# CrystalSixone/VLN-GOAT

Measured on AMD Instinct MI355X. Metric: trajectory-steps/sec fwd+bwd (GOAT pretrain, 36 views x 768, 80 tok), higher is better.
Workload: dtype bf16; 1 GPU; Full R2R GOAT pretrain config (pretrain_src/run_r2r_goat.sh): 6,3,2 layers text/cross/pano, vocab 50265, per-rank batch 48, T=5, 36x768 views, L=80, tasks mlm/sap/cfp 1:1:1, dropout 0.1, fwd+bwd, random-init; global_batch=48, parallelism=dp1, wire=f32, launch=hipGraph replay

## Files before the change

vln-goat_amd/csrc/causal.hip:

```cpp
#include "common.hpp"

namespace {

constexpr int POOL_MAXL = 512;
template <typename T>
__global__ __launch_bounds__(256) void pool_score_kernel(const T* __restrict__ x, const float* __restrict__ w,
                                                         const float* __restrict__ out, const float* __restrict__ dout,
                                                         float* __restrict__ score, int rows, int L, int H,
                                                         const float* __restrict__ smask = nullptr) {
  const int lane = threadIdx.x & 63;
  const int row = blockIdx.x * 4 + (threadIdx.x >> 6);
  if (row >= rows) return;
  const T* xr = x + (int64_t)row * H;
  const int b = row / L;
  float s = 0.f;
  if (out == nullptr) {
    for (int i = lane; i < H; i += 64) s += tanhf(to_f(xr[i])) * w[i];
  } else {
    for (int i = lane; i < H; i += 64) {
      const float o = out[(int64_t)b * H + i];
      s += to_f(xr[i]) * dout[(int64_t)b * H + i] * (1.f - o * o);
    }
  }
  s = wave_sum(s);
// ... 129 lines not shown
    const T* d = dout + (int64_t)row * H;
    const float s = gate[row];
    float dg = 0.f;
    for (int i = lane; i < H; i += 64) dg += to_f(d[i]) * (to_f(a[i]) - to_f(o[i]));
    dg = wave_sum(dg);
    const float dpre = dg * s * (1.f - s);
    pb += dpre;
#pragma unroll
    for (int j = 0; j < DOOR_MAXC; ++j) {
      const int i = lane + 64 * j;
      if (i < H) {
        const float dv = to_f(d[i]), av = to_f(a[i]), ov = to_f(o[i]);
        daug[(int64_t)row * H + i] = from_f<T>(s * dv + dpre * wa[i]);
        dori[(int64_t)row * H + i] = from_f<T>((1.f - s) * dv + dpre * wo[i]);
        pa[j] += dpre * av;
        po[j] += dpre * ov;
      }
    }
  }
#pragma unroll
  for (int j = 0; j < DOOR_MAXC; ++j) {
    const int i = lane + 64 * j;
    if (i < H) { sm[(wave * 2 + 0) * H + i] = pa[j]; sm[(wave * 2 + 1) * H + i] = po[j]; }
  }
  __syncthreads();
  for (int i = threadIdx.x; i < 2 * H; i += 256) {
    const int which = i / H, col = i % H;
    const float v = sm[(0 * 2 + which) * H + col] + sm[(1 * 2 + which) * H + col] + sm[(2 * 2 + which) * H + col] +
                    sm[(3 * 2 + which) * H + col];
    atomicAdd((which ? dwo : dwa) + col, v);
  }
  if (lane == 0) {
    atomicAdd(dbias, pb);
    if (dbias2) atomicAdd(dbias2, pb);
  }
}

template <typename T>
__global__ __launch_bounds__(256) void dict_wsum_fwd_kernel(const float* __restrict__ z, const float* __restrict__ p,
                                                            T* __restrict__ out, int K, int H) {
  const int b = blockIdx.x;
  for (int i = threadIdx.x; i < H; i += 256) {
    float s = 0.f;
    for (int k = 0; k < K; ++k) s += p[(int64_t)b * K + k] * z[((int64_t)b * K + k) * H + i];
    out[(int64_t)b * H + i] = from_f<T>(s);
  }
}
template <typename T>
__global__ __launch_bounds__(256) void dict_wsum_bwd_kernel(const T* __restrict__ dout, const float* __restrict__ z,
                                                            const float* __restrict__ p, float* __restrict__ dz,
                                                            float* __restrict__ dp, int K, int H) {
  const int b = blockIdx.x, lane = threadIdx.x & 63, wave = threadIdx.x >> 6;
  const T* d = dout + (int64_t)b * H;
  if (dz)
    for (int k = 0; k < K; ++k) {
      const float pk = p[(int64_t)b * K + k];
      for (int i = threadIdx.x; i < H; i += 256) dz[((int64_t)b * K + k) * H + i] = pk * to_f(d[i]);
    }
  if (dp)
    for (int k = wave; k < K; k += 4) {
      float s = 0.f;
      for (int i = lane; i < H; i += 64) s += z[((int64_t)b * K + k) * H + i] * to_f(d[i]);
      s = wave_sum(s);
      if (lane == 0) dp[(int64_t)b * K + k] = s;
    }
}


struct NceArgs {
  const float* a[6];
  const float* b[6];
  float* da[6];
  float* db[6];
  float* prob;
  float* loss;
  const float* dloss;
  int Bl, Ba, H, target0;
  float inv_tau;
};

struct NceRole { float* out; int rows; int n; int pd[6]; int is_b[6]; };
struct NceBwdArgs { NceArgs p; NceRole role[8]; int nroles; int row_groups; };

__global__ __launch_bounds__(256) void infonce_fwd_kernel(NceArgs p) {
  extern __shared__ float sh[];
  __shared__ float lsum;
  const int i = blockIdx.x;
  const int lane = threadIdx.x & 63, wave = threadIdx.x >> 6;
  if (threadIdx.x == 0) lsum = 0.f;
  for (int pd = 0; pd < 6; ++pd) {
    const float* arow = p.a[pd] + (int64_t)i * p.H;
    __syncthreads();
    for (int j = wave; j < p.Ba; j += 4) {
      const float* brow = p.b[pd] + (int64_t)j * p.H;
      float s = 0.f;
      for (int k = lane * 4; k < p.H; k += 256) {
        const f32x4 x = *reinterpret_cast<const f32x4*>(arow + k), y = *reinterpret_cast<const f32x4*>(brow + k);
        s += x[0] * y[0] + x[1] * y[1] + x[2] * y[2] + x[3] * y[3];
      }
      s = wave_sum(s);
      if (lane == 0) sh[j] = s * p.inv_tau;
    }
    __syncthreads();
    if (wave == 0) {
      float m = -INFINITY;
      for (int j = lane; j < p.Ba; j += 64) m = fmaxf(m, sh[j]);
      m = wave_max(m);
      float l = 0.f;
      for (int j = lane; j < p.Ba; j += 64) l += __expf(sh[j] - m);
      l = wave_sum(l);
      const float lse = m + __logf(l);
      float* pr = p.prob + ((int64_t)pd * p.Bl + i) * p.Ba;
      for (int j = lane; j < p.Ba; j += 64) pr[j] = __expf(sh[j] - lse);
      if (lane == 0) lsum += 0.5f * (lse - sh[p.target0 + i]);
    }
  }
  __syncthreads();
  if (threadIdx.x == 0) p.loss[i] += lsum;
}

__global__ __launch_bounds__(256) void infonce_bwd_kernel(NceBwdArgs q) {
  const NceArgs& p = q.p;
  const int ro = blockIdx.x / q.row_groups, rg = blockIdx.x % q.row_groups;
  const NceRole& role = q.role[ro];
  const int r = rg * 4 + (threadIdx.x >> 6), c = blockIdx.y * 64 + (threadIdx.x & 63);
  if (r >= role.rows || c >= p.H) return;
  const float half_tau = 0.5f * p.inv_tau;
  float tot = 0.f;
  for (int t = 0; t < role.n; ++t) {
    const int pd = role.pd[t];
    const float* pr = p.prob + (int64_t)pd * p.Bl * p.Ba;
    float acc = 0.f;
    if (!role.is_b[t]) {
      if (r < p.Bl) {
        const float* B = p.b[pd];
        const int tr = p.target0 + r;
        for (int j = 0; j < p.Ba; ++j) acc += (pr[(int64_t)r * p.Ba + j] - (j == tr ? 1.f : 0.f)) * B[(int64_t)j * p.H + c];
        acc *= p.dloss[r] * half_tau;
      }
    } else if (r < p.Ba) {
      const float* A = p.a[pd];
      for (int i = 0; i < p.Bl; ++i)
        acc += (pr[(int64_t)i * p.Ba + r] - (r == p.target0 + i ? 1.f : 0.f)) * (p.dloss[i] * half_tau) * A[(int64_t)i * p.H + c];
    }
    tot += acc;
  }
  role.out[(int64_t)r * p.H + c] += tot;
}


struct SapArgs {
  const void* gs; const void* ls; const void* fwl;
  const uint8_t* gvis; const uint8_t* gvalid; const int64_t* glens; const uint8_t* lmask;
  const float* M; const int64_t* ga; const int64_t* la;
  float* gl; float* ll; float* fused; float* loss; float* lse;
  const float* dloss; const float* dgl; const float* dll; const float* dfused;
  void* dgs; void* dls; void* dfwl;
  int B, G, W, lmask_is_valid, add_stop, fw_sigmoid;
};

__device__ __forceinline__ bool sap_gmasked(const SapArgs& p, int b, int g) {
  bool m = false;
  if (p.gvis) m = m || p.gvis[(int64_t)b * p.G + g] != 0;
  if (p.gvalid) m = m || p.gvalid[(int64_t)b * p.G + g] == 0;
  if (p.glens) m = m || g >= (int)p.glens[b];
  return m;
}
__device__ __forceinline__ bool sap_lmasked(const SapArgs& p, int b, int w) {
  if (!p.lmask) return false;
  const bool v = p.lmask[(int64_t)b * p.W + w] != 0;
  return p.lmask_is_valid ? !v : v;
}
template <typename T>
__device__ __forceinline__ float sap_fw(const SapArgs& p, int b) {
  if (!p.fwl) return 0.5f;
  const float x = (float)reinterpret_cast<const T*>(p.fwl)[b];
  return p.fw_sigmoid ? 1.f / (1.f + __expf(-x)) : x;
}
__device__ __forceinline__ float sap_lse(const float* v, int n, int lane) {
  float m = -INFINITY;
  for (int i = lane; i < n; i += 64) m = fmaxf(m, v[i]);
  m = wave_max(m);
  if (m == -INFINITY) return -INFINITY;
  float s = 0.f;
  for (int i = lane; i < n; i += 64) s += __expf(v[i] - m);
  return m + __logf(wave_sum(s));
}

template <typename T>
__global__ __launch_bounds__(64) void sap_fwd_kernel(SapArgs p) {
  extern __shared__ float sm[];
  float* s_gl = sm; float* s_ll = sm + p.G; float* s_lz = s_ll + p.W; float* s_fu = s_lz + p.W;
  const int b = blockIdx.x, lane = threadIdx.x;
  const float fw = sap_fw<T>(p, b);
  const T* gs = reinterpret_cast<const T*>(p.gs) + (int64_t)b * p.G;
  const T* ls = reinterpret_cast<const T*>(p.ls) + (int64_t)b * p.W;
  for (int g = lane; g < p.G; g += 64) {
    const float v = sap_gmasked(p, b, g) ? -INFINITY : (float)gs[g] * fw;
    s_gl[g] = v;
    p.gl[(int64_t)b * p.G + g] = v;
  }
  for (int w = lane; w < p.W; w += 64) {
    const bool m = sap_lmasked(p, b, w);
    const float r = (float)ls[w] * (1.f - fw);
    s_ll[w] = m ? -INFINITY : r;
    s_lz[w] = m ? 0.f : r;
    p.ll[(int64_t)b * p.W + w] = s_ll[w];
  }
  __syncthreads();
  for (int g = lane; g < p.G; g += 64) {
    float acc = 0.f;
    if (p.M) {
      const float* mr = p.M + ((int64_t)b * p.G + g) * p.W;
      for (int w = 0; w < p.W; ++w) acc += mr[w] * s_lz[w];
    }
    float v = s_gl[g] + acc;
    if (p.add_stop && g == 0) v += s_ll[0];
    s_fu[g] = v;
    p.fused[(int64_t)b * p.G + g] = v;
  }
  __syncthreads();
  if (p.lse) {
    const float lg = sap_lse(s_gl, p.G, lane), lw = sap_lse(s_ll, p.W, lane), lf = sap_lse(s_fu, p.G, lane);
    if (lane == 0) {
      p.lse[b * 3] = lg; p.lse[b * 3 + 1] = lw; p.lse[b * 3 + 2] = lf;
      if (p.loss) {
        const int ga = p.ga ? (int)p.ga[b] : -1, la = p.la ? (int)p.la[b] : -1;
        float l = 0.f;
        if (ga >= 0 && ga < p.G) l += (lg - s_gl[ga]) + (lf - s_fu[ga]);
        if (la >= 0 && la < p.W) l += lw - s_ll[la];
// ... 184 lines not shown
    return 0;
  });
}

extern "C" int goat_door_gate_fwd(void* stream, int dtype, const void* aug, const void* ori, const float* wa,
                                  const float* wo, const float* ba, const float* bo, void* out, float* gate, int rows, int H) {
  if (!aug || !ori || !wa || !wo || !ba || !bo || !out || !gate) return GOAT_E_ARG;
  if (rows <= 0 || H <= 0) return GOAT_E_SHAPE;
  const int blocks = (rows + 3) / 4;
  return dtype_dispatch(dtype, [&](auto dt) -> int {
    typedef GOAT_DT_TYPE(dt) T;
    hipLaunchKernelGGL(door_fwd_kernel<T>, dim3(blocks), dim3(256), 0, ST(stream), (const T*)aug, (const T*)ori, wa, wo, ba, bo,
                       (T*)out, gate, rows, H);
    GOAT_LAUNCH_CHECK();
    return 0;
  });
}

extern "C" int goat_door_gate_bwd(void* stream, int dtype, const void* aug, const void* ori, const float* wa,
                                  const float* wo, const float* gate, const void* dout, void* daug, void* dori, float* dwa,
                                  float* dwo, float* dbias, int rows, int H, float* dbias2) {
  if (!aug || !ori || !wa || !wo || !gate || !dout || !daug || !dori || !dwa || !dwo || !dbias) return GOAT_E_ARG;
  if (rows <= 0 || H <= 0 || H > 64 * DOOR_MAXC) return GOAT_E_SHAPE;
  int blocks = (rows + 3) / 4;
  if (blocks > 256) blocks = 256;
  const size_t sm = (size_t)8 * H * sizeof(float);
  return dtype_dispatch(dtype, [&](auto dt) -> int {
    typedef GOAT_DT_TYPE(dt) T;
    hipLaunchKernelGGL(door_bwd_kernel<T>, dim3(blocks), dim3(256), sm, ST(stream), (const T*)aug, (const T*)ori, wa, wo, gate,
                       (const T*)dout, (T*)daug, (T*)dori, dwa, dwo, dbias, dbias2, rows, H);
    GOAT_LAUNCH_CHECK();
    return 0;
  });
}

extern "C" int goat_dict_wsum_fwd(void* stream, int dtype_out, const float* z, const float* p, void* out, int B, int K,
                                  int H) {
  if (!z || !p || !out) return GOAT_E_ARG;
  if (B <= 0 || K <= 0 || H <= 0) return GOAT_E_SHAPE;
  return dtype_dispatch(dtype_out, [&](auto dt) -> int {
    typedef GOAT_DT_TYPE(dt) T;
    hipLaunchKernelGGL(dict_wsum_fwd_kernel<T>, dim3(B), dim3(256), 0, ST(stream), z, p, (T*)out, K, H);
    GOAT_LAUNCH_CHECK();
    return 0;
  });
}

extern "C" int goat_dict_wsum_bwd(void* stream, int dtype_dout, const void* dout, const float* z, const float* p,
                                  float* dz, float* dp, int B, int K, int H) {
  if (!dout || !z || !p) return GOAT_E_ARG;
  if (B <= 0 || K <= 0 || H <= 0) return GOAT_E_SHAPE;
  if (!dz && !dp) return 0;
  return dtype_dispatch(dtype_dout, [&](auto dt) -> int {
    typedef GOAT_DT_TYPE(dt) T;
    hipLaunchKernelGGL(dict_wsum_bwd_kernel<T>, dim3(B), dim3(256), 0, ST(stream), (const T*)dout, z, p, dz, dp, K, H);
    GOAT_LAUNCH_CHECK();
    return 0;
  });
}

static int nce_fill(NceArgs& a, const float* const* x_loc, const float* const* x_all, const float* txt_loc, const float* txt_all,
                    float* const* dx_loc, float* const* dx_all, float* dtxt_loc, float* dtxt_all, float* prob, int Bl, int Ba, int H,
                    int target0, float temperature) {
  if (!x_loc || !x_all || !txt_loc || !txt_all || !prob) return GOAT_E_ARG;
  if (Bl <= 0 || Ba < Bl || H <= 0 || (H % 4) || target0 < 0 || target0 + Bl > Ba || !(temperature > 0.f)) return GOAT_E_SHAPE;
  for (int k = 0; k < 3; ++k) {
    if (!x_loc[k] || !x_all[k]) return GOAT_E_ARG;
    a.a[2 * k] = x_loc[k]; a.b[2 * k] = txt_all;
    a.a[2 * k + 1] = txt_loc; a.b[2 * k + 1] = x_all[k];
    a.da[2 * k] = dx_loc ? dx_loc[k] : nullptr; a.db[2 * k] = dtxt_all;
    a.da[2 * k + 1] = dtxt_loc; a.db[2 * k + 1] = dx_all ? dx_all[k] : nullptr;
  }
  a.prob = prob; a.Bl = Bl; a.Ba = Ba; a.H = H; a.target0 = target0; a.inv_tau = 1.f / temperature;
  return 0;
}

extern "C" int goat_infonce_fwd(void* stream, const float* const* x_loc, const float* const* x_all, const float* txt_loc,
                                const float* txt_all, float* loss, float* prob, int Bl, int Ba, int H, int target0, float temperature) {
  NceArgs a = {};
  if (!loss) return GOAT_E_ARG;
  if (int e = nce_fill(a, x_loc, x_all, txt_loc, txt_all, nullptr, nullptr, nullptr, nullptr, prob, Bl, Ba, H, target0, temperature)) return e;
  if ((size_t)Ba * 4 > 64 * 1024) return GOAT_E_SHAPE;
  a.loss = loss;
  hipLaunchKernelGGL(infonce_fwd_kernel, dim3(Bl), dim3(256), (size_t)Ba * 4, ST(stream), a);
  GOAT_LAUNCH_CHECK();
  return 0;
}

extern "C" int goat_infonce_bwd(void* stream, const float* const* x_loc, const float* const* x_all, const float* txt_loc,
                                const float* txt_all, const float* dloss, const float* prob, float* const* dx_loc, float* const* dx_all,
                                float* dtxt_loc, float* dtxt_all, int Bl, int Ba, int H, int target0, float temperature) {
  NceArgs a = {};
  if (!dloss) return GOAT_E_ARG;
  if (int e = nce_fill(a, x_loc, x_all, txt_loc, txt_all, dx_loc, dx_all, dtxt_loc, dtxt_all, const_cast<float*>(prob), Bl, Ba, H, target0,
                       temperature))
    return e;
  a.dloss = dloss;
  NceBwdArgs q = {};
  q.p = a;
  for (int pd = 0; pd < 6; ++pd)
    for (int is_b = 0; is_b < 2; ++is_b) {
      float* out = is_b ? a.db[pd] : a.da[pd];
      if (!out) continue;
      int ro = 0;
      while (ro < q.nroles && q.role[ro].out != out) ++ro;
      if (ro == q.nroles) { q.role[ro].out = out; q.role[ro].rows = 0; q.role[ro].n = 0; ++q.nroles; }
      NceRole& role = q.role[ro];
      role.pd[role.n] = pd; role.is_b[role.n] = is_b; ++role.n;
      const int rows = is_b ? Ba : Bl;
      if (rows > role.rows) role.rows = rows;
    }
  if (q.nroles == 0) return 0;
  q.row_groups = (Ba + 3) / 4;
  hipLaunchKernelGGL(infonce_bwd_kernel, dim3(q.nroles * q.row_groups, (H + 63) / 64), dim3(256), 0,
                     ST(stream), q);
  GOAT_LAUNCH_CHECK();
  return 0;
}

extern "C" int goat_rowdot_fwd(void* stream, int dtype, const void* x, const float* w, const float* b, void* y, int M, int H) {
  if (!x || !w || !y) return GOAT_E_ARG;
  if (M <= 0 || H <= 0 || (H % 8)) return GOAT_E_SHAPE;
  const int blocks = (M + 3) / 4;
  return dtype_dispatch(dtype, [&](auto dt) -> int {
    typedef GOAT_DT_TYPE(dt) T;
    hipLaunchKernelGGL(rowdot_fwd_kernel<T>, dim3(blocks), dim3(256), 0, ST(stream), (const T*)x, w, b, (T*)y, M, H);
    GOAT_LAUNCH_CHECK();
    return 0;
  });
}

extern "C" int goat_rowdot_bwd(void* stream, int dtype, const void* x, const float* w, const void* dy, void* dx, float* dw, float* db, int M,
                               int H) {
  if (!x || !w || !dy) return GOAT_E_ARG;
  if (db && !dw) return GOAT_E_ARG;
  if (M <= 0 || H <= 0 || (H % 8)) return GOAT_E_SHAPE;
  if (!dx && !dw) return 0;
  int blocks = (M + 3) / 4;
  if (blocks > 128) blocks = 128;
  const size_t sm = (size_t)4 * H * sizeof(float);
  return dtype_dispatch(dtype, [&](auto dt) -> int {
    typedef GOAT_DT_TYPE(dt) T;
    constexpr int MAXC = sizeof(T) == 2 ? 2 : 4;
    if (H > 64 * dt.EPC * MAXC) return GOAT_E_SHAPE;
    hipLaunchKernelGGL((rowdot_bwd_kernel<T, MAXC>), dim3(blocks), dim3(256), sm, ST(stream), (const T*)x, w, (const T*)dy, (T*)dx, dw, db,
                       M, H);
    GOAT_LAUNCH_CHECK();
    return 0;
  });
}

extern "C" int goat_cfp_mix_fwd(void* stream, int dtype_fwl, const float* go, const float* vo, const void* fwl, float* fo, float* fw, int B, int H) {
  if (!go || !vo || !fwl || !fo || !fw) return GOAT_E_ARG;
  if (B <= 0 || H <= 0) return GOAT_E_SHAPE;
  return dtype_dispatch(dtype_fwl, [&](auto dt) -> int {
    typedef GOAT_DT_TYPE(dt) T;
    hipLaunchKernelGGL(cfp_mix_fwd_kernel<T>, dim3(B), dim3(256), 0, ST(stream), go, vo, (const T*)fwl, fo, fw, H);
    GOAT_LAUNCH_CHECK();
    return 0;
  });
}

extern "C" int goat_cfp_mix_bwd(void* stream, int dtype_fwl, const float* go, const float* vo, const float* fw, const float* dfo, float* dgo,
                                float* dvo, void* dfwl, int B, int H, int accumulate) {
  if (!go || !vo || !fw || !dfo || !dgo || !dvo || !dfwl) return GOAT_E_ARG;
  if (B <= 0 || H <= 0) return GOAT_E_SHAPE;
  return dtype_dispatch(dtype_fwl, [&](auto dt) -> int {
    typedef GOAT_DT_TYPE(dt) T;
    hipLaunchKernelGGL(cfp_mix_bwd_kernel<T>, dim3(B), dim3(256), 0, ST(stream), go, vo, fw, dfo, dgo, dvo, (T*)dfwl, H, accumulate);
    GOAT_LAUNCH_CHECK();
    return 0;
  });
}

static int sap_check(const SapArgs& a, int dtype) {
  if (!a.gs || !a.ls || !a.gl || !a.ll || !a.fused) return GOAT_E_ARG;
  if (dtype != GOAT_BF16 && dtype != GOAT_F32) return GOAT_E_ARG;
  if (a.B <= 0 || a.G <= 0 || a.W <= 0 || (size_t)(2 * a.G + 2 * a.W) * 4 > 64 * 1024) return GOAT_E_SHAPE;
  return 0;
}

extern "C" int goat_sap_fuse_fwd(void* stream, int dtype, const void* gs, const void* ls, const void* fwl, int fw_sigmoid,
                                 const uint8_t* gvis, const uint8_t* gvalid, const int64_t* glens, const uint8_t* lmask,
                                 int lmask_is_valid, const float* M, int add_stop, const int64_t* ga, const int64_t* la, float* gl,
                                 float* ll, float* fused, float* loss, float* lse, int B, int G, int W) {
  SapArgs a = {};
  a.gs = gs; a.ls = ls; a.fwl = fwl; a.fw_sigmoid = fw_sigmoid; a.gvis = gvis; a.gvalid = gvalid; a.glens = glens; a.lmask = lmask;
  a.lmask_is_valid = lmask_is_valid; a.M = M; a.add_stop = add_stop; a.ga = ga; a.la = la; a.gl = gl; a.ll = ll; a.fused = fused;
  a.loss = loss; a.lse = lse; a.B = B; a.G = G; a.W = W;
  if (int e = sap_check(a, dtype)) return e;
  if (loss && !lse) return GOAT_E_ARG;
  const size_t smem = (size_t)(2 * G + 2 * W) * 4;
  return dtype_dispatch(dtype, [&](auto dt) -> int {
    hipLaunchKernelGGL(sap_fwd_kernel<GOAT_DT_TYPE(dt)>, dim3(B), dim3(64), smem, ST(stream), a);
    GOAT_LAUNCH_CHECK();
    return 0;
  });
// ... 23 lines not shown
```

vln-goat_amd/csrc/rowops.hip:

```cpp
#include <cstdlib>
#include "common.hpp"
#include <algorithm>
#include <vector>

namespace {

#ifndef GOAT_LN_ABL
#define GOAT_LN_ABL 0
#endif
constexpr int MAXC_MAX = 8;

template <typename T, int MAXC>
__global__ __launch_bounds__(256) void ln_fwd_kernel(const T* __restrict__ x, const T* __restrict__ res,
                                                     const float* __restrict__ gamma, const float* __restrict__ beta,
                                                     float eps, float p, uint64_t seed, uint64_t offset,
                                                     const uint64_t* __restrict__ rng_dev, T* __restrict__ y, T* __restrict__ zout, float* __restrict__ mean,
                                                     float* __restrict__ rstd, int M, int H, float p_out, uint64_t offset_out,
                                                     const T* __restrict__ post_add) {
  constexpr int EPC = DT<T>::EPC;
  const int lane = threadIdx.x & 63;
  const int row = blockIdx.x * 4 + (threadIdx.x >> 6);
  if (row >= M) return;
  if (rng_dev) seed += *rng_dev;
  const GoatRng rng(seed);
// ... 490 lines not shown
    }
    v.store_stream(y + c * EPC);
  }
  if (blockIdx.x == 0 && threadIdx.x < (n - nchunk * EPC)) {
    const int64_t i = nchunk * EPC + threadIdx.x;
    float v = to_f(x[i]);
    if (drop) v = rng.keep(offset + i, thr) ? v * ks : 0.f;
    if (!BWD && res) v += to_f(res[i]);
    y[i] = from_f<T>(v);
  }
}


template <typename T>
__global__ __launch_bounds__(256) void act_bwd_kernel(const T* __restrict__ dy, const T* __restrict__ u, T* __restrict__ dx,
                                                      int64_t n, int act, float p, uint64_t seed, uint64_t offset,
                                                      const uint64_t* __restrict__ rng_dev) {
  constexpr int EPC = DT<T>::EPC;
  if (rng_dev) seed += *rng_dev;
  const GoatRng rng(seed);
  const uint32_t thr = goat_thr16(p);
  const bool drop = p > 0.f;
  const float ks = drop ? 1.f / (1.f - p) : 1.f;
  const int64_t nchunk = n / EPC;
  for (int64_t c = blockIdx.x * (int64_t)blockDim.x + threadIdx.x; c < nchunk; c += (int64_t)gridDim.x * blockDim.x) {
    Chunk<T> d, uu;
    d.load(dy + c * EPC);
    uu.load(u + c * EPC);
    const uint32_t km = drop ? rng.keep_bits<EPC>(offset + c * EPC, thr) : 0xFFFFFFFFu;
#pragma unroll
    for (int e = 0; e < EPC; ++e) {
      float g = d.v[e];
      if (drop) g = ((km >> e) & 1u) ? g * ks : 0.f;
      g *= (act == 1) ? dgelu_f(uu.v[e]) : (uu.v[e] > 0.f ? 1.f : 0.f);
      d.v[e] = g;
    }
    d.store_stream(dx + c * EPC);
  }
  if (blockIdx.x == 0 && threadIdx.x < (n - nchunk * EPC)) {
    const int64_t i = nchunk * EPC + threadIdx.x;
    float g = to_f(dy[i]);
    const float uv = to_f(u[i]);
    if (drop) g = rng.keep(offset + i, thr) ? g * ks : 0.f;
    g *= (act == 1) ? dgelu_f(uv) : (uv > 0.f ? 1.f : 0.f);
    dx[i] = from_f<T>(g);
  }
}


template <typename T>
__global__ __launch_bounds__(256) void colsum_kernel(const T* __restrict__ x, int64_t ld, int R, int C,
                                                     float* __restrict__ colsum, int rows_per_block) {
  __shared__ float part[4][64];
  const int tx = threadIdx.x & 63, ty = threadIdx.x >> 6;
  const int c = blockIdx.x * 64 + tx;
  const int r0 = blockIdx.y * rows_per_block;
  const int r1 = min(R, r0 + rows_per_block);
  float acc = 0.f;
  if (c < C)
    for (int r = r0 + ty; r < r1; r += 4) acc += to_f(x[(int64_t)r * ld + c]);
  part[ty][tx] = acc;
  __syncthreads();
  if (ty == 0 && c < C) atomicAdd(colsum + c, part[0][tx] + part[1][tx] + part[2][tx] + part[3][tx]);
}


__device__ __forceinline__ float block_reduce_dyn(float v, float* red, bool is_max) {
  v = is_max ? wave_max(v) : wave_sum(v);
  const int wave = threadIdx.x >> 6, lane = threadIdx.x & 63;
  __syncthreads();
  if (lane == 0) red[wave] = v;
  __syncthreads();
  float r = red[0];
  for (int w = 1; w < (int)(blockDim.x >> 6); ++w) r = is_max ? fmaxf(r, red[w]) : r + red[w];
  return r;
}

__global__ __launch_bounds__(256) void ce_fwd_kernel(const float* __restrict__ logits, int64_t ld, int N,
                                                     const int64_t* __restrict__ targets, float* __restrict__ loss,
                                                     float* __restrict__ lse) {
  __shared__ float red[4];
  const int m = blockIdx.x;
  const float* row = logits + (int64_t)m * ld;
  float mx = -INFINITY;
  const int n4 = N >> 2;
  for (int c = threadIdx.x; c < n4; c += 256) {
    const f32x4 v = *reinterpret_cast<const f32x4*>(row + c * 4);
    mx = fmaxf(fmaxf(mx, fmaxf(v[0], v[1])), fmaxf(v[2], v[3]));
  }
  for (int c = n4 * 4 + threadIdx.x; c < N; c += 256) mx = fmaxf(mx, row[c]);
  mx = block_reduce_dyn(mx, red, true);
  float sum = 0.f;
  for (int c = threadIdx.x; c < n4; c += 256) {
    const f32x4 v = *reinterpret_cast<const f32x4*>(row + c * 4);
    sum += __expf(v[0] - mx) + __expf(v[1] - mx) + __expf(v[2] - mx) + __expf(v[3] - mx);
  }
  for (int c = n4 * 4 + threadIdx.x; c < N; c += 256) sum += __expf(row[c] - mx);
  sum = block_reduce_dyn(sum, red, false);
  if (threadIdx.x == 0) {
    const float l = mx + __logf(sum);
    lse[m] = l;
    const int64_t t = targets[m];
    loss[m] = t < 0 ? 0.f : (t < (int64_t)N ? l - row[t] : __builtin_nanf(""));
  }
}

template <typename T>
__global__ __launch_bounds__(256) void ce_bwd_kernel(const float* __restrict__ logits, int64_t ld, int N,
                                                     const int64_t* __restrict__ targets, const float* __restrict__ lse,
                                                     const float* __restrict__ dloss, T* __restrict__ dlogits, int64_t ld_out) {
  const int m = blockIdx.x;
  const float* row = logits + (int64_t)m * ld;
  T* out = dlogits + (int64_t)m * ld_out;
  const int t = (int)targets[m];
  const float l = lse[m], g = t < 0 ? 0.f : (t < N ? dloss[m] : __builtin_nanf(""));
  for (int c = threadIdx.x * 4; c < (int)ld_out; c += 256 * 4) {
    float v[4];
#pragma unroll
    for (int e = 0; e < 4; ++e) {
      const int n = c + e;
      v[e] = (n < N) ? (__expf(row[n] - l) - (n == t ? 1.f : 0.f)) * g : 0.f;
    }
#pragma unroll
    for (int e = 0; e < 4; ++e)
      if (c + e < (int)ld_out) out[c + e] = from_f<T>(v[e]);
  }
}

template <typename T>
__global__ __launch_bounds__(256) void transpose_kernel(const T* __restrict__ in, int64_t ld_in, T* __restrict__ out,
                                                        int64_t ld_out, int R, int C, float* __restrict__ colsum, int RT) {
  __shared__ T tile[64][66];
  __shared__ float csum[4][64];
  const int tx = threadIdx.x & 63, ty = threadIdx.x >> 6;
  const int c0 = blockIdx.y * 64;
  float acc = 0.f;
  for (int t = 0; t < RT; ++t) {
    const int r0 = (blockIdx.x * RT + t) * 64;
    if (r0 >= R && r0 >= (int)ld_out) break;
#pragma unroll 4
    for (int i = ty; i < 64; i += 4) {
      const int r = r0 + i, c = c0 + tx;
      T v = (T)0.f;
      if (r < R && c < C) v = in[(int64_t)r * ld_in + c];
      tile[i][tx] = v;
      acc += to_f(v);
    }
    __syncthreads();
#pragma unroll 4
    for (int i = ty; i < 64; i += 4) {
      const int c = c0 + i, r = r0 + tx;
      if (c < C && r < (int)ld_out) out[(int64_t)c * ld_out + r] = tile[tx][i];
    }
    __syncthreads();
  }
  if (colsum) {
    csum[ty][tx] = acc;
    __syncthreads();
    if (ty == 0 && c0 + tx < C) atomicAdd(colsum + c0 + tx, csum[0][tx] + csum[1][tx] + csum[2][tx] + csum[3][tx]);
  }
}

constexpr int SK_MAXK = 16, SK_BATCH = 8;
template <typename T, int KP, int SK_ROWS>
__global__ __launch_bounds__(256) void wgrad_smallk_kernel(const T* __restrict__ dy, int64_t ld_dy, const T* __restrict__ x,
                                                           int64_t ld_x, int rows, int N, int K, float* __restrict__ dw,
                                                           int64_t ld_dw, float* __restrict__ dbias) {
  __shared__ float sm[4][128][SK_MAXK + 1];
  const int lane = threadIdx.x & 63, wave = __builtin_amdgcn_readfirstlane(threadIdx.x >> 6);
  const int n0 = blockIdx.x * 128 + lane * 2;
  const int r0 = blockIdx.y * SK_ROWS, r1 = min(rows, r0 + SK_ROWS);
  float acc[2][SK_MAXK], bsum[2] = {0.f, 0.f};
#pragma unroll
  for (int k = 0; k < SK_MAXK; ++k) { acc[0][k] = 0.f; acc[1][k] = 0.f; }
  const bool in0 = n0 < N, in1 = n0 + 1 < N;
  for (int rb = r0 + wave * SK_BATCH; rb < r1; rb += 4 * SK_BATCH) {
    constexpr int EPC = DT<T>::EPC, NCH = KP / EPC;
    float d0[SK_BATCH], d1[SK_BATCH], xv[SK_BATCH][KP];
#pragma unroll
    for (int u = 0; u < SK_BATCH; ++u) {
      const int r = rb + u;
      const bool live = r < r1;
      d0[u] = (live && in0) ? to_f(dy[(int64_t)r * ld_dy + n0]) : 0.f;
      d1[u] = (live && in1) ? to_f(dy[(int64_t)r * ld_dy + n0 + 1]) : 0.f;
#pragma unroll
      for (int c = 0; c < NCH; ++c) {
        Chunk<T> ch;
        if (live) ch.load(x + (int64_t)r * ld_x + c * EPC);
#pragma unroll
        for (int e = 0; e < EPC; ++e) xv[u][c * EPC + e] = live ? ch.v[e] : 0.f;
      }
    }
#pragma unroll
    for (int u = 0; u < SK_BATCH; ++u) {
      bsum[0] += d0[u]; bsum[1] += d1[u];
#pragma unroll
      for (int k = 0; k < KP; ++k) {
        acc[0][k] += d0[u] * xv[u][k];
        acc[1][k] += d1[u] * xv[u][k];
      }
    }
  }
#pragma unroll
  for (int c = 0; c < 2; ++c) {
#pragma unroll
    for (int k = 0; k < SK_MAXK; ++k) sm[wave][lane * 2 + c][k] = acc[c][k];
    sm[wave][lane * 2 + c][SK_MAXK] = bsum[c];
  }
  __syncthreads();
// ... 622 lines not shown
}

extern "C" int goat_dropout_add_fwd(void* stream, int dtype, const void* x, const void* residual, void* y, int64_t n,
                                    float p, uint64_t seed, uint64_t offset, const uint64_t* rng_dev) {
  if (!x || !y) return GOAT_E_ARG;
  if (n <= 0) return GOAT_E_SHAPE;
  int64_t blocks = (n / 8 + 255) / 256;
  if (blocks > 2048) blocks = 2048;
  if (blocks < 1) blocks = 1;
  return dtype_dispatch(dtype, [&](auto dt) -> int {
    typedef GOAT_DT_TYPE(dt) T;
    hipLaunchKernelGGL((dropout_kernel<T, false>), dim3((int)blocks), dim3(256), 0, ST(stream), (const T*)x, (const T*)residual, (T*)y, n, p,
                       seed, offset, rng_dev);
    GOAT_LAUNCH_CHECK();
    return 0;
  });
}

extern "C" int goat_dropout_bwd(void* stream, int dtype, const void* dy, void* dx, int64_t n, float p, uint64_t seed,
                                uint64_t offset, const uint64_t* rng_dev) {
  if (!dy || !dx) return GOAT_E_ARG;
  if (n <= 0) return GOAT_E_SHAPE;
  int64_t blocks = (n / 8 + 255) / 256;
  if (blocks > 2048) blocks = 2048;
  if (blocks < 1) blocks = 1;
  return dtype_dispatch(dtype, [&](auto dt) -> int {
    typedef GOAT_DT_TYPE(dt) T;
    hipLaunchKernelGGL((dropout_kernel<T, true>), dim3((int)blocks), dim3(256), 0, ST(stream), (const T*)dy, (const T*)nullptr, (T*)dx, n, p,
                       seed, offset, rng_dev);
    GOAT_LAUNCH_CHECK();
    return 0;
  });
}

extern "C" int goat_act_bwd(void* stream, int dtype, const void* dy, const void* u, void* dx, int64_t n, int act,
                            float p, uint64_t seed, uint64_t offset, const uint64_t* rng_dev) {
  if (!dy || !u || !dx) return GOAT_E_ARG;
  if (n <= 0) return GOAT_E_SHAPE;
  if (act != GOAT_EPI_GELU && act != GOAT_EPI_RELU) return GOAT_E_ARG;
  int64_t blocks = (n / 8 + 255) / 256;
  if (blocks > 2048) blocks = 2048;
  if (blocks < 1) blocks = 1;
  return dtype_dispatch(dtype, [&](auto dt) -> int {
    typedef GOAT_DT_TYPE(dt) T;
    hipLaunchKernelGGL(act_bwd_kernel<T>, dim3((int)blocks), dim3(256), 0, ST(stream), (const T*)dy, (const T*)u, (T*)dx, n, act, p, seed,
                       offset, rng_dev);
    GOAT_LAUNCH_CHECK();
    return 0;
  });
}

extern "C" int goat_colsum(void* stream, int dtype, const void* x, int64_t ld, int R, int C, float* colsum) {
  if (!x || !colsum) return GOAT_E_ARG;
  if (R <= 0 || C <= 0) return GOAT_E_SHAPE;
  const int cb = (C + 63) / 64;
  int rb = (1024 + cb - 1) / cb;
  if (rb > (R + 31) / 32) rb = (R + 31) / 32;
  if (rb < 1) rb = 1;
  const int rows_per_block = (R + rb - 1) / rb;
  dim3 grid(cb, (R + rows_per_block - 1) / rows_per_block);
  return dtype_dispatch(dtype, [&](auto dt) -> int {
    typedef GOAT_DT_TYPE(dt) T;
    hipLaunchKernelGGL(colsum_kernel<T>, grid, dim3(256), 0, ST(stream), (const T*)x, ld, R, C, colsum, rows_per_block);
    GOAT_LAUNCH_CHECK();
    return 0;
  });
}

extern "C" int goat_ce_fwd(void* stream, const float* logits, int64_t ld, int M, int N, const int64_t* targets,
                           float* loss, float* lse) {
  if (!logits || !targets || !loss || !lse) return GOAT_E_ARG;
  if (M <= 0 || N <= 0 || ld < N || (ld & 3) || (reinterpret_cast<uintptr_t>(logits) & 15)) return GOAT_E_SHAPE;
  hipLaunchKernelGGL(ce_fwd_kernel, dim3(M), dim3(256), 0, ST(stream), logits, ld, N, targets, loss, lse);
  GOAT_LAUNCH_CHECK();
  return 0;
}

extern "C" int goat_ce_bwd(void* stream, int dtype_out, const float* logits, int64_t ld, int M, int N,
                           const int64_t* targets, const float* lse, const float* dloss, void* dlogits, int64_t ld_out) {
  if (!logits || !targets || !lse || !dloss || !dlogits) return GOAT_E_ARG;
  if (M <= 0 || N <= 0 || ld < N || ld_out < N) return GOAT_E_SHAPE;
  return dtype_dispatch(dtype_out, [&](auto dt) -> int {
    typedef GOAT_DT_TYPE(dt) T;
    hipLaunchKernelGGL(ce_bwd_kernel<T>, dim3(M), dim3(256), 0, ST(stream), logits, ld, N, targets, lse, dloss, (T*)dlogits, ld_out);
    GOAT_LAUNCH_CHECK();
    return 0;
  });
}

extern "C" int goat_transpose(void* stream, int dtype, const void* in, int64_t ld_in, void* out, int64_t ld_out, int R,
                              int C, float* colsum) {
  if (!in || !out) return GOAT_E_ARG;
  if (R <= 0 || C <= 0 || ld_out < R || ld_in < C) return GOAT_E_SHAPE;
  const int rtiles = (int)((ld_out + 63) / 64), ctiles = (C + 63) / 64;
  int RT = 1;
  while (RT < 16 && (int64_t)((rtiles + 2 * RT - 1) / (2 * RT)) * ctiles >= 1024) RT *= 2;
  dim3 grid((rtiles + RT - 1) / RT, ctiles);
  return dtype_dispatch(dtype, [&](auto dt) -> int {
    typedef GOAT_DT_TYPE(dt) T;
    hipLaunchKernelGGL(transpose_kernel<T>, grid, dim3(256), 0, ST(stream), (const T*)in, ld_in, (T*)out, ld_out, R, C, colsum, RT);
    GOAT_LAUNCH_CHECK();
    return 0;
  });
}

extern "C" int goat_wgrad_smallk(void* stream, int dtype, const void* dy, int64_t ld_dy, const void* x, int64_t ld_x, int rows,
                                 int N, int K, float* dw, int64_t ld_dw, float* dbias) {
  if (!dy || !x || !dw) return GOAT_E_ARG;
  if (rows <= 0 || N <= 0 || K <= 0 || K > SK_MAXK) return GOAT_E_SHAPE;
  const int rc = rows >= 2048 ? 128 : 32;
  dim3 grid((N + 127) / 128, (rows + rc - 1) / rc);
  const int epc = dtype == GOAT_BF16 ? 8 : 4, kp = (K + epc - 1) / epc * epc;
  if (ld_x < kp || (ld_x % epc) || (reinterpret_cast<uintptr_t>(x) & 15)) return GOAT_E_SHAPE;
#define GOAT_SK_LAUNCH(T_, KP_)                                                                                              \
  do {                                                                                                                       \
    if (rc == 128)                                                                                                           \
      hipLaunchKernelGGL((wgrad_smallk_kernel<T_, KP_, 128>), grid, dim3(256), 0, ST(stream), (const T_*)dy, ld_dy, (const T_*)x, ld_x, \
                         rows, N, K, dw, ld_dw, dbias);                                                                      \
    else                                                                                                                     \
      hipLaunchKernelGGL((wgrad_smallk_kernel<T_, KP_, 32>), grid, dim3(256), 0, ST(stream), (const T_*)dy, ld_dy, (const T_*)x, ld_x, \
                         rows, N, K, dw, ld_dw, dbias);                                                                      \
  } while (0)
  if (dtype == GOAT_BF16) {
    if (kp == 8) GOAT_SK_LAUNCH(bf16_t, 8); else GOAT_SK_LAUNCH(bf16_t, 16);
  } else if (dtype == GOAT_F32) {
    if (kp == 4) GOAT_SK_LAUNCH(float, 4); else if (kp == 8) GOAT_SK_LAUNCH(float, 8);
    else if (kp == 12) GOAT_SK_LAUNCH(float, 12); else GOAT_SK_LAUNCH(float, 16);
  } else {
    return GOAT_E_ARG;
  }
#undef GOAT_SK_LAUNCH
  GOAT_LAUNCH_CHECK();
  return 0;
}

extern "C" int goat_pano_fusion_fwd(void* stream, int dtype, const void* x, const float* a, const float* a0, void* fused,
                                    float* wsave, int N, int V, int H) {
  if (!x || !a || !a0 || !fused || !wsave) return GOAT_E_ARG;
  if (N <= 0 || V <= 0 || V > 64 || H <= 0) return GOAT_E_SHAPE;
  size_t sm = (size_t)PF_NW * H * sizeof(float);
#ifdef GOAT_PANO_GENERIC
  sm = 1 << 30;
#endif
  return dtype_dispatch(dtype, [&](auto dt) -> int {
    typedef GOAT_DT_TYPE(dt) T;
    constexpr int MC = sizeof(T) == 2 ? 2 : 3;
    if (H % dt.EPC == 0 && H <= 64 * dt.EPC * MC && sm <= 64 * 1024)
      hipLaunchKernelGGL((pano_fusion_fwd_kernel<T, MC>), dim3(N), dim3(64 * PF_NW), sm, ST(stream), (const T*)x, a, a0, (T*)fused, wsave, V, H);
    else
      hipLaunchKernelGGL(pano_fusion_fwd_generic<T>, dim3(N), dim3(256), 0, ST(stream), (const T*)x, a, a0, (T*)fused, wsave, V, H);
    GOAT_LAUNCH_CHECK();
    return 0;
  });
}

extern "C" int goat_pano_fusion_bwd(void* stream, int dtype, const void* x, const float* a, const float* a0,
                                    const float* wsave, const void* dfused, void* dx, float* da, float* da0, int N,
                                    int V, int H) {
  if (!x || !a || !a0 || !wsave || !dfused || !dx || !da || !da0) return GOAT_E_ARG;
  if (N <= 0 || V <= 0 || V > 64 || H <= 0) return GOAT_E_SHAPE;
  size_t sm = (size_t)PF_NW * H * sizeof(float);
#ifdef GOAT_PANO_GENERIC
  sm = 1 << 30;
#endif
  return dtype_dispatch(dtype, [&](auto dt) -> int {
    typedef GOAT_DT_TYPE(dt) T;
    constexpr int MC = sizeof(T) == 2 ? 2 : 3;
// ... 100 lines not shown
```

Measured before the change: 48870 trajectory-steps/s.

## Parallelize InfoNCE fwd/bwd across pairs and use online-softmax CE kernels

Adds a 768-thread InfoNCE forward kernel that processes all six pairs at once, two waves per pair, with four B rows per iteration. It rewrites the InfoNCE backward so each wave handles one pair term and broadcasts gradients via readlane, reusing each X load across four rows, then reduces the partials in shared memory. Cross-entropy forward becomes a single-pass online max/sum, and a vectorized chunked cross-entropy backward kernel is added for aligned inputs. The goal is fewer serial passes and better memory reuse, at the cost of more code paths and slightly different floating-point rounding.

```diff
diff --git a/vln-goat_amd/csrc/causal.hip b/vln-goat_amd/csrc/causal.hip
--- a/vln-goat_amd/csrc/causal.hip
+++ b/vln-goat_amd/csrc/causal.hip
@@ -235,6 +235,76 @@
 struct NceRole { float* out; int rows; int n; int pd[6]; int is_b[6]; };
 struct NceBwdArgs { NceArgs p; NceRole role[8]; int nroles; int row_groups; };
 
+__device__ __forceinline__ float nce_dot4(float s, const f32x4& x, const f32x4& y) {
+#pragma clang fp contract(off)
+  const float t = x[0] * y[0] + x[1] * y[1] + x[2] * y[2] + x[3] * y[3];
+  return s + t;
+}
+
+constexpr int NCE_FAST_MAXBA = 2048;
+__global__ __launch_bounds__(768) void infonce_fwd_wide_kernel(NceArgs p) {
+  extern __shared__ float sh[];
+  __shared__ float term[6];
+  const int i = blockIdx.x;
+  const int lane = threadIdx.x & 63, wave = threadIdx.x >> 6;
+  const int pd = wave >> 1, half = wave & 1;
+  const int Ba = p.Ba, H = p.H;
+  float* s_pd = sh + pd * Ba;
+  const float* arow = p.a[pd] + (int64_t)i * H;
+  const float* bmat = p.b[pd];
+  int j = half;
+  for (; j + 6 < Ba; j += 8) {
+    const float* b0 = bmat + (int64_t)j * H;
+    const float* b1 = b0 + 2 * (int64_t)H;
+    const float* b2 = b0 + 4 * (int64_t)H;
+    const float* b3 = b0 + 6 * (int64_t)H;
+    float s0 = 0.f, s1 = 0.f, s2 = 0.f, s3 = 0.f;
+    for (int k = lane * 4; k < H; k += 256) {
+      const f32x4 x = *reinterpret_cast<const f32x4*>(arow + k);
+      const f32x4 y0 = *reinterpret_cast<const f32x4*>(b0 + k), y1 = *reinterpret_cast<const f32x4*>(b1 + k);
+      const f32x4 y2 = *reinterpret_cast<const f32x4*>(b2 + k), y3 = *reinterpret_cast<const f32x4*>(b3 + k);
+      s0 = nce_dot4(s0, x, y0);
+      s1 = nce_dot4(s1, x, y1);
+      s2 = nce_dot4(s2, x, y2);
+      s3 = nce_dot4(s3, x, y3);
+    }
+    s0 = wave_sum(s0); s1 = wave_sum(s1); s2 = wave_sum(s2); s3 = wave_sum(s3);
+    if (lane == 0) {
+      s_pd[j] = s0 * p.inv_tau; s_pd[j + 2] = s1 * p.inv_tau; s_pd[j + 4] = s2 * p.inv_tau; s_pd[j + 6] = s3 * p.inv_tau;
+    }
+  }
+  for (; j < Ba; j += 2) {
+    const float* brow = bmat + (int64_t)j * H;
+    float s = 0.f;
+    for (int k = lane * 4; k < H; k += 256) {
+      const f32x4 x = *reinterpret_cast<const f32x4*>(arow + k), y = *reinterpret_cast<const f32x4*>(brow + k);
+      s = nce_dot4(s, x, y);
+    }
+    s = wave_sum(s);
+    if (lane == 0) s_pd[j] = s * p.inv_tau;
+  }
+  __syncthreads();
+  if (half == 0) {
+    float m = -INFINITY;
+    for (int jj = lane; jj < Ba; jj += 64) m = fmaxf(m, s_pd[jj]);
+    m = wave_max(m);
+    float l = 0.f;
+    for (int jj = lane; jj < Ba; jj += 64) l += __expf(s_pd[jj] - m);
+    l = wave_sum(l);
+    const float lse = m + __logf(l);
+    float* pr = p.prob + ((int64_t)pd * p.Bl + i) * Ba;
+    for (int jj = lane; jj < Ba; jj += 64) pr[jj] = __expf(s_pd[jj] - lse);
+    if (lane == 0) term[pd] = 0.5f * (lse - s_pd[p.target0 + i]);
+  }
+  __syncthreads();
+  if (threadIdx.x == 0) {
+    float lsum = 0.f;
+#pragma unroll
+    for (int k = 0; k < 6; ++k) lsum += term[k];
+    p.loss[i] += lsum;
+  }
+}
+
 __global__ __launch_bounds__(256) void infonce_fwd_kernel(NceArgs p) {
   extern __shared__ float sh[];
   __shared__ float lsum;
@@ -249,7 +319,7 @@
       float s = 0.f;
       for (int k = lane * 4; k < p.H; k += 256) {
         const f32x4 x = *reinterpret_cast<const f32x4*>(arow + k), y = *reinterpret_cast<const f32x4*>(brow + k);
-        s += x[0] * y[0] + x[1] * y[1] + x[2] * y[2] + x[3] * y[3];
+        s = nce_dot4(s, x, y);
       }
       s = wave_sum(s);
       if (lane == 0) sh[j] = s * p.inv_tau;
@@ -272,33 +342,73 @@
   if (threadIdx.x == 0) p.loss[i] += lsum;
 }
 
-__global__ __launch_bounds__(256) void infonce_bwd_kernel(NceBwdArgs q) {
+constexpr int NCE_BWD_WAVES = 6;
+__device__ __forceinline__ float nce_lane(float v, int l) { return __int_as_float(__builtin_amdgcn_readlane(__float_as_int(v), l)); }
+__global__ __launch_bounds__(64 * NCE_BWD_WAVES) void infonce_bwd_kernel(NceBwdArgs q) {
+  __shared__ float part[NCE_BWD_WAVES][4][64];
   const NceArgs& p = q.p;
   const int ro = blockIdx.x / q.row_groups, rg = blockIdx.x % q.row_groups;
   const NceRole& role = q.role[ro];
-  const int r = rg * 4 + (threadIdx.x >> 6), c = blockIdx.y * 64 + (threadIdx.x & 63);
-  if (r >= role.rows || c >= p.H) return;
+  if (rg * 4 >= role.rows) return;
+  const int lane = threadIdx.x & 63, t = threadIdx.x >> 6;
+  const int c = blockIdx.y * 64 + lane;
+  const int cl = c < p.H ? c : p.H - 1;
+  const int r0 = rg * 4;
   const float half_tau = 0.5f * p.inv_tau;
-  float tot = 0.f;
-  for (int t = 0; t < role.n; ++t) {
+  if (t < role.n) {
     const int pd = role.pd[t];
+    const bool is_b = role.is_b[t] != 0;
     const float* pr = p.prob + (int64_t)pd * p.Bl * p.Ba;
-    float acc = 0.f;
-    if (!role.is_b[t]) {
-      if (r < p.Bl) {
-        const float* B = p.b[pd];
-        const int tr = p.target0 + r;
-        for (int j = 0; j < p.Ba; ++j) acc += (pr[(int64_t)r * p.Ba + j] - (j == tr ? 1.f : 0.f)) * B[(int64_t)j * p.H + c];
-        acc *= p.dloss[r] * half_tau;
+    const float* X = (is_b ? p.a[pd] : p.b[pd]) + cl;
+    const int n = is_b ? p.Bl : p.Ba;
+    const int nlive = is_b ? p.Ba : p.Bl;
+    float acc[4] = {0.f, 0.f, 0.f, 0.f};
+    for (int j0 = 0; j0 < n; j0 += 64) {
+      const int cnt = n - j0 < 64 ? n - j0 : 64;
+      float g[4] = {0.f, 0.f, 0.f, 0.f};
+      if (lane < cnt) {
+        const int j = j0 + lane;
+        const float sc = is_b ? p.dloss[j] * half_tau : 0.f;
+#pragma unroll
+        for (int k = 0; k < 4; ++k) {
+          const int r = r0 + k;
+          if (r < nlive)
+            g[k] = is_b ? (pr[(int64_t)j * p.Ba + r] - (r == p.target0 + j ? 1.f : 0.f)) * sc
+                        : pr[(int64_t)r * p.Ba + j] - (j == p.target0 + r ? 1.f : 0.f);
+        }
       }
-    } else if (r < p.Ba) {
-      const float* A = p.a[pd];
-      for (int i = 0; i < p.Bl; ++i)
-        acc += (pr[(int64_t)i * p.Ba + r] - (r == p.target0 + i ? 1.f : 0.f)) * (p.dloss[i] * half_tau) * A[(int64_t)i * p.H + c];
-    }
-    tot += acc;
-  }
-  role.out[(int64_t)r * p.H + c] += tot;
+      const float* Xj = X + (int64_t)j0 * p.H;
+      int jj = 0;
+      for (; jj + 16 <= cnt; jj += 16) {
+        float x[16];
+#pragma unroll
+        for (int u = 0; u < 16; ++u) x[u] = Xj[(int64_t)(jj + u) * p.H];
+#pragma unroll
+        for (int u = 0; u < 16; ++u)
+#pragma unroll
+          for (int k = 0; k < 4; ++k) acc[k] = fmaf(nce_lane(g[k], jj + u), x[u], acc[k]);
+      }
+      for (; jj < cnt; ++jj) {
+        const float x = Xj[(int64_t)jj * p.H];
+#pragma unroll
+        for (int k = 0; k < 4; ++k) acc[k] = fmaf(nce_lane(g[k], jj), x, acc[k]);
+      }
+    }
+#pragma unroll
+    for (int k = 0; k < 4; ++k) {
+      const int r = r0 + k;
+      if (r >= nlive) acc[k] = 0.f;
+      else if (!is_b) acc[k] *= p.dloss[r] * half_tau;
+      part[t][k][lane] = acc[k];
+    }
+  }
+  __syncthreads();
+  if (t < 4) {
+    const int r = r0 + t;
+    float tot = 0.f;
+    for (int k = 0; k < role.n; ++k) tot += part[k][t][lane];
+    if (r < role.rows && c < p.H) role.out[(int64_t)r * p.H + c] += tot;
+  }
 }
 
 
@@ -649,7 +759,8 @@
   if (int e = nce_fill(a, x_loc, x_all, txt_loc, txt_all, nullptr, nullptr, nullptr, nullptr, prob, Bl, Ba, H, target0, temperature)) return e;
   if ((size_t)Ba * 4 > 64 * 1024) return GOAT_E_SHAPE;
   a.loss = loss;
-  hipLaunchKernelGGL(infonce_fwd_kernel, dim3(Bl), dim3(256), (size_t)Ba * 4, ST(stream), a);
+  if (Ba <= NCE_FAST_MAXBA) hipLaunchKernelGGL(infonce_fwd_wide_kernel, dim3(Bl), dim3(768), (size_t)6 * Ba * 4, ST(stream), a);
+  else hipLaunchKernelGGL(infonce_fwd_kernel, dim3(Bl), dim3(256), (size_t)Ba * 4, ST(stream), a);
   GOAT_LAUNCH_CHECK();
   return 0;
 }
@@ -679,7 +790,7 @@
     }
   if (q.nroles == 0) return 0;
   q.row_groups = (Ba + 3) / 4;
-  hipLaunchKernelGGL(infonce_bwd_kernel, dim3(q.nroles * q.row_groups, (H + 63) / 64), dim3(256), 0,
+  hipLaunchKernelGGL(infonce_bwd_kernel, dim3(q.nroles * q.row_groups, (H + 63) / 64), dim3(64 * NCE_BWD_WAVES), 0,
                      ST(stream), q);
   GOAT_LAUNCH_CHECK();
   return 0;
diff --git a/vln-goat_amd/csrc/rowops.hip b/vln-goat_amd/csrc/rowops.hip
--- a/vln-goat_amd/csrc/rowops.hip
+++ b/vln-goat_amd/csrc/rowops.hip
@@ -596,23 +596,31 @@
   __shared__ float red[4];
   const int m = blockIdx.x;
   const float* row = logits + (int64_t)m * ld;
-  float mx = -INFINITY;
+  float mx = -INFINITY, sum = 0.f;
   const int n4 = N >> 2;
-  for (int c = threadIdx.x; c < n4; c += 256) {
-    const f32x4 v = *reinterpret_cast<const f32x4*>(row + c * 4);
-    mx = fmaxf(fmaxf(mx, fmaxf(v[0], v[1])), fmaxf(v[2], v[3]));
-  }
-  for (int c = n4 * 4 + threadIdx.x; c < N; c += 256) mx = fmaxf(mx, row[c]);
+  auto take = [&](const f32x4& v) {
+    const float cm = fmaxf(fmaxf(v[0], v[1]), fmaxf(v[2], v[3]));
+    if (cm > mx) { sum *= __expf(mx - cm); mx = cm; }
+    const float ms = mx == -INFINITY ? 0.f : mx;
+    sum += __expf(v[0] - ms) + __expf(v[1] - ms) + __expf(v[2] - ms) + __expf(v[3] - ms);
+  };
+  int c = threadIdx.x;
+  for (; c + 768 < n4; c += 1024) {
+    const f32x4 v0 = *reinterpret_cast<const f32x4*>(row + c * 4), v1 = *reinterpret_cast<const f32x4*>(row + (c + 256) * 4);
+    const f32x4 v2 = *reinterpret_cast<const f32x4*>(row + (c + 512) * 4), v3 = *reinterpret_cast<const f32x4*>(row + (c + 768) * 4);
+    take(v0); take(v1); take(v2); take(v3);
+  }
+  for (; c < n4; c += 256) take(*reinterpret_cast<const f32x4*>(row + c * 4));
+  for (int k = n4 * 4 + threadIdx.x; k < N; k += 256) {
+    const float v = row[k];
+    if (v > mx) { sum *= __expf(mx - v); mx = v; }
+    sum += __expf(v - (mx == -INFINITY ? 0.f : mx));
+  }
+  const float own = mx;
   mx = block_reduce_dyn(mx, red, true);
-  float sum = 0.f;
-  for (int c = threadIdx.x; c < n4; c += 256) {
-    const f32x4 v = *reinterpret_cast<const f32x4*>(row + c * 4);
-    sum += __expf(v[0] - mx) + __expf(v[1] - mx) + __expf(v[2] - mx) + __expf(v[3] - mx);
-  }
-  for (int c = n4 * 4 + threadIdx.x; c < N; c += 256) sum += __expf(row[c] - mx);
-  sum = block_reduce_dyn(sum, red, false);
+  sum = block_reduce_dyn(sum * __expf(own - (mx == -INFINITY ? 0.f : mx)), red, false);
   if (threadIdx.x == 0) {
-    const float l = mx + __logf(sum);
+    const float l = mx == -INFINITY ? __builtin_nanf("") : mx + __logf(sum);
     lse[m] = l;
     const int64_t t = targets[m];
     loss[m] = t < 0 ? 0.f : (t < (int64_t)N ? l - row[t] : __builtin_nanf(""));
@@ -639,6 +647,43 @@
     for (int e = 0; e < 4; ++e)
       if (c + e < (int)ld_out) out[c + e] = from_f<T>(v[e]);
   }
+}
+
+template <typename T>
+__global__ __launch_bounds__(256) void ce_bwd_wide_kernel(const float* __restrict__ logits, int64_t ld, int N,
+                                                          const int64_t* __restrict__ targets, const float* __restrict__ lse,
+                                                          const float* __restrict__ dloss, T* __restrict__ dlogits, int64_t ld_out) {
+  constexpr int EPC = DT<T>::EPC;
+  const int m = blockIdx.x;
+  const float* row = logits + (int64_t)m * ld;
+  T* out = dlogits + (int64_t)m * ld_out;
+  const int t = (int)targets[m];
+  const float l = lse[m], g = t < 0 ? 0.f : (t < N ? dloss[m] : __builtin_nanf(""));
+  const int npieces = (int)(ld_out / EPC);
+  auto piece = [&](int pc) {
+    const int c = pc * EPC;
+    Chunk<T> o;
+    if (c + EPC <= N && (t < c || t >= c + EPC)) {
+      float v[EPC];
+#pragma unroll
+      for (int e = 0; e < EPC; e += 4) {
+        const f32x4 x = *reinterpret_cast<const f32x4*>(row + c + e);
+        v[e] = x[0]; v[e + 1] = x[1]; v[e + 2] = x[2]; v[e + 3] = x[3];
+      }
+#pragma unroll
+      for (int e = 0; e < EPC; ++e) o.v[e] = __expf(v[e] - l) * g;
+    } else {
+#pragma unroll
+      for (int e = 0; e < EPC; ++e) {
+        const int n = c + e;
+        o.v[e] = (n < N) ? (__expf(row[n] - l) - (n == t ? 1.f : 0.f)) * g : 0.f;
+      }
+    }
+    o.store(out + c);
+  };
+  int pc = threadIdx.x;
+  for (; pc + 256 < npieces; pc += 512) { piece(pc); piece(pc + 256); }
+  if (pc < npieces) piece(pc);
 }
 
 template <typename T>
@@ -1427,7 +1472,9 @@
   if (M <= 0 || N <= 0 || ld < N || ld_out < N) return GOAT_E_SHAPE;
   return dtype_dispatch(dtype_out, [&](auto dt) -> int {
     typedef GOAT_DT_TYPE(dt) T;
-    hipLaunchKernelGGL(ce_bwd_kernel<T>, dim3(M), dim3(256), 0, ST(stream), logits, ld, N, targets, lse, dloss, (T*)dlogits, ld_out);
+    const bool wide = !((reinterpret_cast<uintptr_t>(logits) | reinterpret_cast<uintptr_t>(dlogits)) & 15) && !(ld & 3) && !(ld_out % dt.EPC);
+    if (wide) hipLaunchKernelGGL(ce_bwd_wide_kernel<T>, dim3(M), dim3(256), 0, ST(stream), logits, ld, N, targets, lse, dloss, (T*)dlogits, ld_out);
+    else hipLaunchKernelGGL(ce_bwd_kernel<T>, dim3(M), dim3(256), 0, ST(stream), logits, ld, N, targets, lse, dloss, (T*)dlogits, ld_out);
     GOAT_LAUNCH_CHECK();
     return 0;
   });
```

Result: no change. 49360 trajectory-steps/s (median of 6 runs) (+1.0%).
